# KhutornoyYaroslav/vcm-ts

Measured on AMD Instinct MI355X. Metric: encoded frames/sec at 1920x1080 GOP-32, higher is better.
Workload: dtype f32 (fp16x3 split-MFMA, fp32 accumulate)

## Files before the change

include/dcvc_hip.h:

```cpp
#ifndef DCVC_HIP_H
#define DCVC_HIP_H

#include <stdint.h>

#ifdef __cplusplus
extern "C" {
#endif

#define DCVC_OK 0
#define DCVC_E_ARG (-1)
#define DCVC_E_LAUNCH (-2)
#define DCVC_E_RANGE (-3)

#define DCVC_STATUS_ACT_SATURATED 1

#define DCVC_MAX_SEG 3

#define DCVC_PREC_FP32 0
#define DCVC_PREC_FP16X3 1

typedef struct {
    const float *ptr;
    int32_t C;
    int32_t cs;
} dcvc_seg;

typedef struct {
    dcvc_seg seg[DCVC_MAX_SEG];
    int32_t nseg;
    int32_t N, Hin, Win;
    int32_t in_act;
    float in_slope;
    const float *wpack;
    const float *bpack;
    int32_t ks;
    int32_t stride;
    int32_t Cout;
    int32_t Cout_pad;
    float *out;
    int32_t out_cs;
    int32_t out_act;
    float out_slope;
    int32_t pixel_shuffle;
    const float *res;
    int32_t res_cs;
    const float *res_gate;
    const float *res2;
    int32_t res2_cs;
    int32_t precision;
    int32_t *status;
    float *chan_partial;
    int32_t tile_row0;
    int32_t tile_rows;
    int32_t pair_taps;
} dcvc_conv_args;

int32_t dcvc_conv_tile_rows(int32_t ks, int32_t stride);

int32_t dcvc_conv_chan_partial_parts(int32_t ks, int32_t stride, int32_t Hout, int32_t Wout);
int dcvc_channel_mean_finish(const float *chan_partial, int32_t parts, int32_t row_stride, float *mean, int32_t N,
                             int32_t C, int32_t HW, void *stream);

int64_t dcvc_conv_pack_size(int32_t Cout, int32_t ks, int32_t nseg, const int32_t *seg_C, int32_t *cout_pad);

int dcvc_conv_pack_weights(const float *w, const float *b, int32_t Cout, int32_t ks, int32_t nseg,
                           const int32_t *seg_C, int32_t pixel_shuffle, int32_t precision, float *wpack,
                           float *bpack);

int64_t dcvc_conv_pack_size_paired(int32_t Cout, int32_t Cin, int32_t *cout_pad);
int dcvc_conv_pack_weights_paired(const float *w, const float *b, int32_t Cout, int32_t Cin, float *wpack, float *bpack);

int dcvc_conv2d(const dcvc_conv_args *a, void *stream);
int dcvc_conv_set_lookahead(int32_t mode);

int64_t dcvc_conv_small_pack_bytes(int32_t Cout, int32_t ks, int32_t nseg, const int32_t *seg_C);
int dcvc_conv_small_pack_weights(const float *w, const float *b, int32_t Cout, int32_t ks, int32_t nseg,
                                 const int32_t *seg_C, void *wpack, float *bpack);
int dcvc_conv2d_small(const dcvc_conv_args *a, void *stream);

int64_t dcvc_conv_k32_pack_bytes(int32_t Cout, int32_t ks, int32_t nseg, const int32_t *seg_C, int32_t *cout_pad);
int dcvc_conv_k32_pack_weights(const float *w, const float *b, int32_t Cout, int32_t ks, int32_t nseg,
                               const int32_t *seg_C, int32_t pixel_shuffle, void *wpack, float *bpack);
int dcvc_conv2d_k32(const dcvc_conv_args *a, void *stream);
int dcvc_conv_k32_set_waves(int32_t waves);

int dcvc_warp(const float *src, int32_t src_cs, const float *flow, int32_t flow_cs, float *out, int32_t out_cs,
              int32_t N, int32_t H, int32_t W, int32_t C, void *stream);
int dcvc_up2(const float *src, int32_t src_cs, float *out, int32_t out_cs, float *out2, int32_t out2_cs,
             int32_t N, int32_t H, int32_t W, int32_t C, float scale, void *stream);
int dcvc_down2(const float *src, int32_t src_cs, float *out, int32_t out_cs, int32_t N, int32_t H, int32_t W,
               int32_t C, float scale, int32_t avgpool_order, void *stream);
int dcvc_maxpool2(const float *src, int32_t src_cs, float *out, int32_t out_cs, int32_t N, int32_t H, int32_t W,
                  int32_t C, void *stream);
int dcvc_copy_channels(const float *src, int32_t src_cs, float *out, int32_t out_cs, int64_t npix, int32_t C,
                       void *stream);
int dcvc_nchw_to_nhwc(const float *src, float *out, int32_t out_cs, int32_t N, int32_t C, int32_t H, int32_t W,
                      void *stream);
int dcvc_nhwc_to_nchw(const float *src, int32_t src_cs, float *out, int32_t N, int32_t C, int32_t H, int32_t W,
                      int32_t clamp01, void *stream);

int dcvc_channel_mean(const float *src, int32_t src_cs, float *mean, float *scratch, int32_t N, int32_t HW,
                      int32_t C, void *stream);
int dcvc_se_gate(const float *mean, const float *w1, const float *w2, float *gate, int32_t N, int32_t C,
                 int32_t Cr, void *stream);

int dcvc_scale_channels(const float *src, int32_t src_cs, float *out, int32_t out_cs, const float *q_basic,
                        const float *q_scale, int32_t mode, int32_t N, int32_t HW, int32_t C, void *stream);
int dcvc_scale_channels_map(const float *src, int32_t src_cs, float *out, int32_t out_cs, const float *q_basic,
                            const float *q_scale, int32_t mode, int32_t N, int32_t HW, int32_t C, const float *q_map,
                            int32_t H, int32_t W, void *stream);
int dcvc_round_symbols(const float *z, int32_t z_cs, float *z_hat, int32_t zh_cs, int32_t *sym, int32_t N,
                       int32_t H, int32_t W, int32_t C, void *stream);
int dcvc_symbols_to_nhwc(const int32_t *sym, float *out, int32_t out_cs, int32_t N, int32_t H, int32_t W,
                         int32_t C, void *stream);

typedef struct {
    const float *y;
    int32_t y_cs;
    const float *fusion;
    int32_t fusion_cs;
    const float *spatial;
    int32_t spatial_cs;
    float *params;
    int32_t params_cs;
    float *y_hat;
    float *y_q;
    float *y_res;
    float *scales_hat;
    int32_t *sym;
    int32_t *idx;
    float *out;
    int32_t out_cs;
    const float *q_basic;
    const float *q_scale;
    int32_t N, H, W, C;
    int32_t step;
    const float *idx_edges;
    const float *forced_q;
    const float *q_map;
} dcvc_dual_prior_args;

int dcvc_scale_indexes(const float *scales, int32_t *idx, int64_t n, const float *idx_edges, void *stream);

int dcvc_dual_prior_enc(const dcvc_dual_prior_args *a, void *stream);
int dcvc_dual_prior_dec_index(const dcvc_dual_prior_args *a, void *stream);
int dcvc_dual_prior_dec_apply(const dcvc_dual_prior_args *a, void *stream);

int dcvc_scale_bits(const float *y_q, const float *scales_hat, float *out, float *scratch, int32_t kind, int32_t N,
                    int64_t per_sample, void *stream);
int dcvc_factorized_bits(const float *z_hat, int32_t z_cs, const float *params, float *out, float *scratch, int32_t N,
                         int32_t HW, int32_t C, void *stream);
int dcvc_sq_err(const float *a, int32_t a_cs, const float *b, int32_t b_cs, float *out, float *scratch, int32_t N,
                int32_t HW, int32_t C, void *stream);

int32_t dcvc_cdf_table_cols(void);
int dcvc_build_scale_cdfs(const float *scales, int32_t n_scales, int32_t kind, int32_t *cdf, int32_t *sizes,
                          int32_t *offsets, void *stream);
int dcvc_build_factorized_cdfs(const float *params, int32_t C, int32_t *cdf, int32_t *sizes, int32_t *offsets, void *stream);

const char *dcvc_hip_version(void);

#ifdef __cplusplus
}
#endif
#endif
```

vcm_ts_amd/csrc/conv_k32.hip:

```cpp
#include <hip/hip_runtime.h>
#include <math.h>
#include <stdint.h>
#include <stdlib.h>
#include <string.h>

#include "dcvc_hip.h"
#include "kernel_common.h"


namespace {

constexpr int KC = 32;
constexpr int REC = 40;

struct K32 {
    const float *seg_ptr[DCVC_MAX_SEG];
    int seg_C[DCVC_MAX_SEG];
    int seg_cs[DCVC_MAX_SEG];
    int nseg;
    int H, W;
    int in_act;
    float in_slope;
    const float *wpack;
    const float *bpack;
    int Cout, Cout_pad;
    float *out;
    int out_cs;
    int out_act;
    float out_slope;
    int ps;
    const float *res;
    int res_cs;
    const float *res_gate;
    const float *res2;
    int res2_cs;
    int *status;
    float *chan_partial;
    int ntx;
    int ty0, nty, band_rows;
};

template <int KS, int NTW, int NWAVE>
__global__ __launch_bounds__(64 * NWAVE, NWAVE / 2) void conv_k32(const K32 a) {
    constexpr int NTH = 64 * NWAVE, RW = 8 / NWAVE, MT = 2 * RW;

    constexpr int BH = 8, BW = 32, BN = 16 * NTW;
    constexpr int PH = BH + KS - 1, PW = BW + KS - 1, PAD = KS / 2;
    constexpr int T = KS * KS, TPS = KS, NST = KS;
    constexpr int LDS_MAIN = PH * PW * REC + TPS * 8 * BN * 4;
    static_assert(LDS_MAIN >= 8 * BN, "the SE reduction reuses the front of the buffer");
    __shared__ __attribute__((aligned(16))) float lds[LDS_MAIN];
    float *patch = lds;
    float *wl = lds + PH * PW * REC;

    const int tid = threadIdx.x, lane = tid & 63, wave = tid >> 6;
    const int nbn = a.Cout_pad / BN;
    const int nb = blockIdx.x % nbn, tx = blockIdx.x / nbn;
    const int ty = blockIdx.y + a.ty0;
    const int x0 = tx * BW, y0 = ty * BH, n0 = nb * BN, img = blockIdx.z;

    f32x4 acc[MT][NTW];
#pragma unroll
    for (int m = 0; m < MT; ++m)
#pragma unroll
        for (int n = 0; n < NTW; ++n) acc[m][n] = (f32x4){0.f, 0.f, 0.f, 0.f};

    const int a_base = ((wave * RW) * PW + (lane & 15)) * REC + (lane >> 4) * 4;
    const int b_base = ((lane >> 4) * BN + (lane & 15)) * 4;

    constexpr int NP = (PH * PW * 8 + NTH - 1) / NTH, NW = (TPS * 8 * BN + NTH - 1) / NTH;
    f32x4 rp[NP], rw[NW];
    struct Cursor {
        int s, c0, cg, st;
    };
    auto advance = [&](Cursor &k) {
        if (++k.st == NST) {
            k.st = 0;
            ++k.cg;
            k.c0 += KC;
            if (k.c0 >= a.seg_C[k.s]) {
                ++k.s;
                k.c0 = 0;
            }
        }
    };
    static_assert((PH * PW * 241 < (1 << 23) && PW == 34) || KS != 3, "the multiply-shift below divides by PW = 34");
    auto ld16 = [](const void *base, unsigned byte_off) __attribute__((always_inline)) {
        return *(const f32x4 *)((const char *)base + byte_off);
    };
    static_assert((PH * PW) % 4 == 0, "slot_pixel permutes inside groups of four pixels");
    auto slot_pixel = [](int q) __attribute__((always_inline)) { return (q & ~3) | ((q & 1) << 1) | ((q >> 1) & 1); };
    auto load_patch = [&](const Cursor &k) {
        const unsigned cs4 = (unsigned)a.seg_cs[k.s] * 4u;
        const char *sp = (const char *)(a.seg_ptr[k.s] + (size_t)img * a.H * a.W * a.seg_cs[k.s] + k.c0);
        int t = tid;
        asm volatile("" : "+v"(t));
        const unsigned lane_off = (t & 7) * 16u;
        const unsigned img_bytes = (unsigned)(a.H * a.W) * cs4;
        const __amdgpu_buffer_rsrc_t rs = __builtin_amdgcn_make_buffer_rsrc((void *)sp, 0, (int)img_bytes, 0x00020000);
#pragma unroll
        for (int u = 0; u < NP; ++u) {
            const int i = t + u * NTH;
            const int p = slot_pixel(i >> 3);
            const int py = PW == 34 ? (p * 241) >> 13 : p / PW, px = p - py * PW;
            const int gy = y0 - PAD + py, gx = x0 - PAD + px;
            const unsigned ok = (unsigned)(tid + u * NTH < PH * PW * 8) & (unsigned)((unsigned)gy < (unsigned)a.H) &
                                (unsigned)((unsigned)gx < (unsigned)a.W);
            const unsigned off = ok ? __umul24((unsigned)(gy * a.W + gx), cs4) + lane_off : img_bytes;
            rp[u] = __builtin_bit_cast(f32x4, __builtin_amdgcn_raw_buffer_load_b128(rs, (int)off, 0, 0));
        }
    };
    auto store_patch = [&]() {
#pragma unroll
        for (int u = 0; u < NP; ++u) {
            const int i = tid + u * NTH;
            if (i < PH * PW * 8) {
                f32x4 sv = rp[u] * ACT_SCALE;
                if (a.in_act) {
#pragma unroll
                    for (int e = 0; e < 4; ++e) {
                        const float t = sv[e] * a.in_slope;
                        float r;
                        asm("v_max_f32 %0, %1, %2" : "=v"(r) : "v"(sv[e]), "v"(t));
                        sv[e] = r;
                    }
                }
#pragma unroll
                for (int e = 0; e < 4; ++e) sv[e] = __builtin_amdgcn_fmed3f(sv[e], -F16_MAX, F16_MAX);
                const f16x4 hi = __builtin_convertvector(sv, f16x4);
                const f16x4 lo = __builtin_convertvector(sv - __builtin_convertvector(hi, f32x4), f16x4);
                _Float16 *rec = (_Float16 *)&patch[slot_pixel(i >> 3) * REC];
                *(f16x4 *)&rec[(i & 7) * 4] = hi;
                *(f16x4 *)&rec[32 + (i & 7) * 4] = lo;
            }
        }
    };
    auto load_w = [&](const Cursor &k) {
        const char *wsrc = (const char *)(a.wpack + ((size_t)(k.cg * T + k.st * TPS) * 8) * a.Cout_pad * 4 + (size_t)n0 * 4);
        int t = tid;
        asm volatile("" : "+v"(t));
#pragma unroll
        for (int u = 0; u < NW; ++u) {
            const int i = t + u * NTH;
            if (u + 1 < NW || tid + u * NTH < TPS * 8 * BN) rw[u] = ld16(wsrc, (unsigned)((i / BN) * a.Cout_pad + (i % BN)) * 16u);
        }
    };
    auto store_w = [&]() {
#pragma unroll
        for (int u = 0; u < NW; ++u) {
            const int i = tid + u * NTH;
            if (i < TPS * 8 * BN) *(f32x4 *)&wl[i * 4] = rw[u];
        }
    };

    auto mfma_step = [&](int st) __attribute__((always_inline)) {
        const int a_st = st * PW * REC;
#pragma unroll
        for (int tl = 0; tl < TPS; ++tl) {
            f16x8 ah[MT], al[MT], bh[NTW], bl[NTW];
#pragma unroll
            for (int m = 0; m < MT; ++m) {
                const float *rec = &patch[a_base + a_st + ((m >> 1) * PW + (m & 1) * 16 + tl) * REC];
                ah[m] = *(const f16x8 *)rec;
                al[m] = *(const f16x8 *)(rec + 16);
            }
#pragma unroll
            for (int n = 0; n < NTW; ++n) {
                bh[n] = *(const f16x8 *)&wl[b_base + ((tl * 2 + 0) * 4 * BN + n * 16) * 4];
                bl[n] = *(const f16x8 *)&wl[b_base + ((tl * 2 + 1) * 4 * BN + n * 16) * 4];
            }
#pragma unroll
            for (int m = 0; m < MT; ++m)
#pragma unroll
                for (int n = 0; n < NTW; ++n) {
                    acc[m][n] = __builtin_amdgcn_mfma_f32_16x16x32_f16(bh[n], ah[m], acc[m][n], 0, 0, 0);
                    acc[m][n] = __builtin_amdgcn_mfma_f32_16x16x32_f16(bl[n], ah[m], acc[m][n], 0, 0, 0);
                    acc[m][n] = __builtin_amdgcn_mfma_f32_16x16x32_f16(bh[n], al[m], acc[m][n], 0, 0, 0);
                }
        }
    };

    Cursor cur = {0, 0, 0, 0};
    load_patch(cur);
    load_w(cur);
    while (cur.s < a.nseg) {
        __syncthreads();
        if (cur.st == 0) store_patch();
        store_w();
        __syncthreads();
        Cursor nxt = cur;
        advance(nxt);
        if (cur.st == 0) {
            Cursor nc = cur;
            nc.c0 += KC;
            if (nc.c0 >= a.seg_C[nc.s]) {
                ++nc.s;
                nc.c0 = 0;
            }
            if (nc.s < a.nseg) load_patch(nc);
        }
        if (nxt.s < a.nseg) load_w(nxt);
        mfma_step(cur.st);
        cur = nxt;
    }

    const int Cq = a.Cout >> 2;
    const int Cfin = a.ps ? Cq : a.Cout;
    const int Ho = a.ps ? a.H * 2 : a.H, Wo = a.ps ? a.W * 2 : a.W;
    constexpr float inv_scale = 1.f / (ACT_SCALE * WGT_SCALE);
    int oy[MT], ox[MT];
    unsigned okm = 0;
#pragma unroll
    for (int m = 0; m < MT; ++m) {
        oy[m] = y0 + wave * RW + (m >> 1);
        ox[m] = x0 + (m & 1) * 16 + (lane & 15);
#pragma unroll
        for (int n = 0; n < NTW; ++n)
            if (oy[m] < a.H && ox[m] < a.W && n0 + n * 16 + (lane >> 4) * 4 < a.Cout) okm |= 1u << (m * NTW + n);
    }
    unsigned pixo[MT];
#pragma unroll
    for (int m = 0; m < MT; ++m) pixo[m] = a.ps ? (unsigned)((2 * oy[m]) * Wo + 2 * ox[m]) : (unsigned)(oy[m] * a.W + ox[m]);
    unsigned chq[NTW], pso[NTW];
#pragma unroll
    for (int n = 0; n < NTW; ++n) {
        const int ch = n0 + n * 16 + (lane >> 4) * 4;
        const int sub = a.ps ? ch / Cq : 0;
        chq[n] = (unsigned)(ch - sub * Cq);
        pso[n] = (unsigned)((sub >> 1) * Wo + (sub & 1));
    }
    auto out_off = [&](int m, int n, int cs) __attribute__((always_inline)) -> unsigned {
        return (__umul24(pixo[m] + pso[n], (unsigned)cs) + chq[n]) * 4u;
    };
    const size_t img_pix = (size_t)img * Ho * Wo;
    const char *res_b = a.res ? (const char *)(a.res + img_pix * a.res_cs) : nullptr;
    const char *res2_b = a.res2 ? (const char *)(a.res2 + img_pix * a.res2_cs) : nullptr;
    char *out_b = (char *)(a.out + img_pix * a.out_cs);
    f32x4 rv[MT][NTW];
    const unsigned out_bytes = (unsigned)(Ho * Wo) * (unsigned)a.out_cs * 4u, res_bytes = (unsigned)(Ho * Wo) * (unsigned)a.res_cs * 4u;
    const __amdgpu_buffer_rsrc_t rs_out = __builtin_amdgcn_make_buffer_rsrc((void *)out_b, 0, (int)out_bytes, 0x00020000);
    const __amdgpu_buffer_rsrc_t rs_res = __builtin_amdgcn_make_buffer_rsrc((void *)res_b, 0, a.res ? (int)res_bytes : 0, 0x00020000);
    if (a.res) {
#pragma unroll
        for (int m = 0; m < MT; ++m)
#pragma unroll
            for (int n = 0; n < NTW; ++n) {
                const bool ok = (okm >> (m * NTW + n)) & 1u;
                rv[m][n] = __builtin_bit_cast(f32x4, __builtin_amdgcn_raw_buffer_load_b128(rs_res, (int)(ok ? out_off(m, n, a.res_cs) : res_bytes), 0, 0));
            }
    }
    f32x4 csum[RW][NTW];
    float vmax = 0.f;
#pragma unroll
    for (int n = 0; n < NTW; ++n) {
#pragma unroll
        for (int r = 0; r < RW; ++r) csum[r][n] = (f32x4){0.f, 0.f, 0.f, 0.f};
        const int ch = n0 + n * 16 + (lane >> 4) * 4;
        const f32x4 bias = *(const f32x4 *)&a.bpack[ch];
        f32x4 gate = {1.f, 1.f, 1.f, 1.f};
        if (a.res_gate && ch < a.Cout) gate = *(const f32x4 *)&a.res_gate[(size_t)img * Cfin + (a.ps ? ch % Cq : ch)];
#pragma unroll
        for (int m = 0; m < MT; ++m) {
            f32x4 v = acc[m][n] * inv_scale + bias;
            if (a.out_act == 1) {
                v[0] = act(v[0], a.out_slope);
                v[1] = act(v[1], a.out_slope);
                v[2] = act(v[2], a.out_slope);
                v[3] = act(v[3], a.out_slope);
            } else if (a.out_act == 2) {
#pragma unroll
                for (int e = 0; e < 4; ++e) v[e] = fminf(fmaxf(v[e], 0.f), 1.f);
            }
            if (a.res) {
                if (a.res_gate) {
#pragma unroll
                    for (int e = 0; e < 4; ++e) v[e] = __builtin_fmaf(rv[m][n][e], gate[e], v[e]);
                } else {
                    v = v + rv[m][n];
                }
            }
            const bool ok = (okm >> (m * NTW + n)) & 1u;
            if (!a.res2 && !a.chan_partial) {
                const float m4 = fmaxf(fmaxf(fabsf(v[0]), fabsf(v[1])), fmaxf(fabsf(v[2]), fabsf(v[3])));
                vmax = fmaxf(vmax, ok ? m4 : 0.f);
                __builtin_amdgcn_raw_buffer_store_b128(__builtin_bit_cast(__attribute__((ext_vector_type(4))) int, v), rs_out,
                                                       (int)(ok ? out_off(m, n, a.out_cs) : out_bytes), 0, 0);
            } else if (ok) {
                if (a.res2) v = ld16(res2_b, out_off(m, n, a.res2_cs)) + v;
                if (a.chan_partial) csum[m >> 1][n] += v;
                vmax = fmaxf(vmax, fmaxf(fmaxf(fabsf(v[0]), fabsf(v[1])), fmaxf(fabsf(v[2]), fabsf(v[3]))));
                *(f32x4 *)(out_b + out_off(m, n, a.out_cs)) = v;
            }
        }
    }
    if (a.status && !(vmax <= ACT_LIMIT)) atomicOr(a.status, DCVC_STATUS_ACT_SATURATED);
    if (a.chan_partial) {
#pragma unroll
        for (int r = 0; r < RW; ++r)
#pragma unroll
            for (int n = 0; n < NTW; ++n)
#pragma unroll
                for (int off = 1; off < 16; off <<= 1)
#pragma unroll
                    for (int e = 0; e < 4; ++e) csum[r][n][e] += __shfl_xor(csum[r][n][e], off);
        float *red = lds;
        __syncthreads();
        if ((lane & 15) == 0)
#pragma unroll
            for (int r = 0; r < RW; ++r)
#pragma unroll
                for (int n = 0; n < NTW; ++n) *(f32x4 *)&red[(wave * RW + r) * BN + n * 16 + (lane >> 4) * 4] = csum[r][n];
        __syncthreads();
        if (tid < BN && n0 + tid < a.Cout_pad) {
            float s = red[tid];
#pragma unroll
            for (int w = 1; w < BH; ++w) s += red[w * BN + tid];
            const size_t part = (size_t)img * (a.nty * a.ntx) + (size_t)ty * a.ntx + tx;
            a.chan_partial[part * a.Cout_pad + n0 + tid] = s;
        }
    }
}

template <int KS, int NTW, int NWAVE>
int launch(K32 &k, int N, hipStream_t st) {
    constexpr int BN = 16 * NTW;
    k.ntx = (k.W + 31) / 32;
    k.nty = (k.H + 7) / 8;
    if (k.ty0 < 0 || k.ty0 >= k.nty) return DCVC_E_ARG;
    const int rows = k.band_rows > 0 ? (k.band_rows < k.nty - k.ty0 ? k.band_rows : k.nty - k.ty0) : k.nty;
    dim3 grid((unsigned)(k.ntx * (k.Cout_pad / BN)), (unsigned)rows, (unsigned)N);
    hipLaunchKernelGGL((conv_k32<KS, NTW, NWAVE>), grid, dim3(64 * NWAVE), 0, st, k);
    RET_LAUNCH();
}

int g_k32_waves = 8;

}

extern "C" int64_t dcvc_conv_k32_pack_bytes(int32_t Cout, int32_t ks, int32_t nseg, const int32_t *seg_C, int32_t *cout_pad) {
    if (Cout <= 0 || nseg <= 0 || nseg > DCVC_MAX_SEG || (ks != 1 && ks != 3)) return DCVC_E_ARG;
    int chunks = 0;
    for (int s = 0; s < nseg; ++s) {
        if (seg_C[s] <= 0 || seg_C[s] % KC) return DCVC_E_ARG;
        chunks += seg_C[s] / KC;
    }
    const int cp = round_up(Cout, 32);
    if (cout_pad) *cout_pad = cp;
    return (int64_t)chunks * ks * ks * 8 * cp * 16;
}

extern "C" int dcvc_conv_k32_pack_weights(const float *w, const float *b, int32_t Cout, int32_t ks, int32_t nseg,
                                          const int32_t *seg_C, int32_t pixel_shuffle, void *wpack, float *bpack) {
    int32_t cp = 0;
    const int64_t total = dcvc_conv_k32_pack_bytes(Cout, ks, nseg, seg_C, &cp);
    if (total < 0 || (pixel_shuffle && (Cout & 3))) return DCVC_E_ARG;
    const int T = ks * ks;
    int Cin = 0;
    for (int s = 0; s < nseg; ++s) Cin += seg_C[s];
    memset(wpack, 0, (size_t)total);
    memset(bpack, 0, (size_t)cp * sizeof(float));
    _Float16 *base = (_Float16 *)wpack;
    const int Cq = Cout / 4;
    bool clamped = false;
    for (int c = 0; c < Cin; ++c) {
        const int cg = c / KC, kq = (c % KC) >> 3, j = c & 7;
        for (int t = 0; t < T; ++t)
            for (int n = 0; n < Cout; ++n) {
                const int np = pixel_shuffle ? ps_packed_channel(n, Cq) : n;
                float sv = w[((size_t)n * Cin + c) * T + t] * WGT_SCALE;
                if (!(fabsf(sv) <= F16_MAX)) { clamped = true; sv = sv > 0.f ? F16_MAX : -F16_MAX; }
                const SplitF16 p = split_f16(sv);
                base[(((((size_t)cg * T + t) * 2 + 0) * 4 + kq) * cp + np) * 8 + j] = p.hi;
                base[(((((size_t)cg * T + t) * 2 + 1) * 4 + kq) * cp + np) * 8 + j] = p.lo;
            }
    }
    for (int n = 0; n < Cout; ++n) bpack[pixel_shuffle ? ps_packed_channel(n, Cq) : n] = b ? b[n] : 0.f;
    return clamped ? DCVC_E_RANGE : DCVC_OK;
}

extern "C" int dcvc_conv_k32_set_waves(int32_t waves) {
    if (waves != 4 && waves != 8) return DCVC_E_ARG;
    g_k32_waves = waves;
    return DCVC_OK;
}

extern "C" int dcvc_conv2d_k32(const dcvc_conv_args *a, void *stream) {
    if (!conv_args_ok(a)) return DCVC_E_ARG;
    if (a->stride != 1 || (a->ks != 1 && a->ks != 3) || a->precision != DCVC_PREC_FP16X3) return DCVC_E_ARG;
    if (a->Cout_pad % 32 || a->Cout > a->Cout_pad || (a->pixel_shuffle && (a->Cout & 3))) return DCVC_E_ARG;
    if (a->out_act < 0 || a->out_act > 2) return DCVC_E_ARG;
    for (int s = 0; s < a->nseg; ++s)
        if (a->seg[s].C <= 0 || a->seg[s].C % KC) return DCVC_E_ARG;
    {
        const unsigned long long opix = (unsigned long long)a->Hin * a->Win * (a->pixel_shuffle ? 4 : 1);
        if (opix >= (1ull << 24) || (unsigned long long)a->out_cs * 4ull >= (1ull << 24) ||
            (a->res && (unsigned long long)a->res_cs * 4ull >= (1ull << 24)) ||
            (a->res2 && (unsigned long long)a->res2_cs * 4ull >= (1ull << 24)))
            return DCVC_E_ARG;
        for (int s = 0; s < a->nseg; ++s)
            if ((unsigned long long)a->seg[s].cs * 4ull >= (1ull << 24)) return DCVC_E_ARG;
        if (opix * a->out_cs * 4ull > 0xfffffff0ull || (a->res && opix * a->res_cs * 4ull > 0xfffffff0ull) ||
            (a->res2 && opix * a->res2_cs * 4ull > 0xfffffff0ull))
            return DCVC_E_ARG;
    }
    if (a->in_act && !(a->in_slope >= 0.f && a->in_slope <= 1.f)) return DCVC_E_ARG;
    for (int s = 0; s < a->nseg; ++s)
        if ((unsigned long long)a->Hin * a->Win * a->seg[s].cs * 4ull > 0xfffffff0ull) return DCVC_E_ARG;
    if (!vec_epilogue_ok(a)) return DCVC_E_ARG;
    if (a->chan_partial && a->pixel_shuffle) return DCVC_E_ARG;
    K32 k;
    memset(&k, 0, sizeof(k));
    copy_conv_args_full(k, a);
    k.H = a->Hin;
    k.W = a->Win;
    hipStream_t st = (hipStream_t)stream;
    const bool wide = (a->Cout_pad % 64) == 0;
    const bool w8 = g_k32_waves != 4;
    if (a->ks == 3) return wide ? (w8 ? launch<3, 4, 8>(k, a->N, st) : launch<3, 4, 4>(k, a->N, st)) : launch<3, 2, 4>(k, a->N, st);
    return wide ? launch<1, 4, 4>(k, a->N, st) : launch<1, 2, 4>(k, a->N, st);
}
```

vcm_ts_amd/lib.py:

```python
from __future__ import annotations

import ctypes as C
import functools
import os

HERE = os.path.dirname(os.path.abspath(__file__))
CSRC = os.path.join(HERE, "csrc")


class LibraryMissing(RuntimeError):
    pass


class KernelError(RuntimeError):
    pass


def _load(name):
    path = os.environ.get("DCVC_HIP_LIB") if name == "libdcvc_hip.so" and os.environ.get("DCVC_HIP_LIB") else \
        os.path.join(CSRC, name)
    if not os.path.exists(path):
        raise LibraryMissing(f"{path} not built; run `make -C {CSRC}` (no CPU fallback exists)")
    return C.CDLL(path)


@functools.lru_cache(maxsize=None)
def rans():
    L = _load("libdcvc_rans.so")
    L.dcvc_rans_encoder_create.restype = C.c_void_p
    L.dcvc_rans_encoder_destroy.argtypes = [C.c_void_p]
    L.dcvc_rans_encoder_reset.argtypes = [C.c_void_p]
    L.dcvc_rans_encoder_encode_with_indexes.argtypes = [C.c_void_p, C.c_void_p, C.c_void_p, C.c_int64, C.c_void_p,
                                                        C.c_int32, C.c_int32, C.c_void_p, C.c_void_p]
    L.dcvc_rans_encoder_flush_bound.argtypes = [C.c_void_p]
    L.dcvc_rans_encoder_flush_bound.restype = C.c_int64
    L.dcvc_rans_encoder_flush.argtypes = [C.c_void_p, C.c_void_p, C.c_int64]
    L.dcvc_rans_encoder_flush.restype = C.c_int64
    L.dcvc_rans_decoder_create.restype = C.c_void_p
    L.dcvc_rans_decoder_destroy.argtypes = [C.c_void_p]
    L.dcvc_rans_decoder_set_stream.argtypes = [C.c_void_p, C.c_char_p, C.c_int64]
    L.dcvc_rans_decoder_decode_stream.argtypes = [C.c_void_p, C.c_void_p, C.c_int64, C.c_void_p, C.c_int32,
                                                  C.c_int32, C.c_void_p, C.c_void_p, C.c_void_p]
    L.dcvc_pmf_to_quantized_cdf.argtypes = [C.c_void_p, C.c_int32, C.c_int32, C.c_void_p]
    return L


class Seg(C.Structure):
    _fields_ = [("ptr", C.c_void_p), ("C", C.c_int32), ("cs", C.c_int32)]


class ConvArgs(C.Structure):
    _fields_ = [
        ("seg", Seg * 3), ("nseg", C.c_int32), ("N", C.c_int32), ("Hin", C.c_int32), ("Win", C.c_int32),
        ("in_act", C.c_int32), ("in_slope", C.c_float), ("wpack", C.c_void_p), ("bpack", C.c_void_p),
        ("ks", C.c_int32), ("stride", C.c_int32), ("Cout", C.c_int32), ("Cout_pad", C.c_int32),
        ("out", C.c_void_p), ("out_cs", C.c_int32), ("out_act", C.c_int32), ("out_slope", C.c_float),
        ("pixel_shuffle", C.c_int32), ("res", C.c_void_p), ("res_cs", C.c_int32), ("res_gate", C.c_void_p),
        ("res2", C.c_void_p), ("res2_cs", C.c_int32), ("precision", C.c_int32), ("status", C.c_void_p),
        ("chan_partial", C.c_void_p), ("tile_row0", C.c_int32), ("tile_rows", C.c_int32), ("pair_taps", C.c_int32),
    ]


class DualPriorArgs(C.Structure):
    _fields_ = [
        ("y", C.c_void_p), ("y_cs", C.c_int32), ("fusion", C.c_void_p), ("fusion_cs", C.c_int32),
        ("spatial", C.c_void_p), ("spatial_cs", C.c_int32), ("params", C.c_void_p), ("params_cs", C.c_int32),
        ("y_hat", C.c_void_p), ("y_q", C.c_void_p), ("y_res", C.c_void_p), ("scales_hat", C.c_void_p),
        ("sym", C.c_void_p), ("idx", C.c_void_p), ("out", C.c_void_p), ("out_cs", C.c_int32),
        ("q_basic", C.c_void_p), ("q_scale", C.c_void_p), ("N", C.c_int32), ("H", C.c_int32), ("W", C.c_int32),
        ("C", C.c_int32), ("step", C.c_int32), ("idx_edges", C.c_void_p), ("forced_q", C.c_void_p),
        ("q_map", C.c_void_p),
    ]


class ConvBwdArgs(C.Structure):
    _fields_ = [
        ("dout", C.c_void_p), ("dout_cs", C.c_int32), ("out", C.c_void_p), ("out_cs", C.c_int32),
        ("res", C.c_void_p), ("res_cs", C.c_int32), ("gate", C.c_void_p), ("res2", C.c_void_p), ("res2_cs", C.c_int32),
        ("dres", C.c_void_p), ("dres_cs", C.c_int32), ("dres2", C.c_void_p), ("dres2_cs", C.c_int32),
        ("dpre", C.c_void_p), ("dpre_cs", C.c_int32), ("zs", C.c_int32), ("Hd", C.c_int32), ("Wd", C.c_int32),
        ("N", C.c_int32), ("Ho", C.c_int32), ("Wo", C.c_int32), ("Cout", C.c_int32), ("pixel_shuffle", C.c_int32),
        ("act", C.c_int32), ("slope", C.c_float),
    ]


class WgradArgs(C.Structure):
    _fields_ = [
        ("x", C.c_void_p), ("x_cs", C.c_int32), ("C", C.c_int32), ("in_act", C.c_int32), ("in_slope", C.c_float),
        ("dpre", C.c_void_p), ("dpre_cs", C.c_int32), ("zs", C.c_int32), ("Hd", C.c_int32), ("Wd", C.c_int32),
        ("N", C.c_int32), ("Hin", C.c_int32), ("Win", C.c_int32), ("Ho", C.c_int32), ("Wo", C.c_int32),
        ("Cout", C.c_int32), ("ks", C.c_int32), ("stride", C.c_int32), ("dw", C.c_void_p), ("Cin_total", C.c_int32),
        ("cin_offset", C.c_int32), ("scratch", C.c_void_p), ("scratch_floats", C.c_int64), ("overwrite", C.c_int32),
        ("db", C.c_void_p), ("precision", C.c_int32),
    ]


class PackJob(C.Structure):
    _fields_ = [
        ("w", C.c_void_p), ("b", C.c_void_p), ("Cout", C.c_int32), ("Cin_total", C.c_int32), ("ks", C.c_int32),
        ("nseg", C.c_int32), ("seg_C", C.c_int32 * 3), ("cin_offset", C.c_int32), ("pixel_shuffle", C.c_int32),
        ("precision", C.c_int32), ("transposed", C.c_int32), ("wpack", C.c_void_p), ("bpack", C.c_void_p),
    ]


class DualPriorBwdArgs(C.Structure):
    _fields_ = [
        ("y", C.c_void_p), ("y_cs", C.c_int32), ("fusion", C.c_void_p), ("fusion_cs", C.c_int32),
        ("y_hat", C.c_void_p), ("dout", C.c_void_p), ("dout_cs", C.c_int32), ("dy_res", C.c_void_p),
        ("dscales_hat", C.c_void_p), ("dparams", C.c_void_p), ("dparams_cs", C.c_int32),
        ("dspatial", C.c_void_p), ("dspatial_cs", C.c_int32), ("dy", C.c_void_p), ("dy_cs", C.c_int32),
        ("dfusion", C.c_void_p), ("dfusion_cs", C.c_int32), ("dq_plane", C.c_void_p),
        ("q_basic", C.c_void_p), ("q_scale", C.c_void_p), ("N", C.c_int32), ("H", C.c_int32), ("W", C.c_int32),
        ("C", C.c_int32), ("step", C.c_int32),
    ]


class ColorCoeffs(C.Structure):
    _fields_ = [(n, C.c_float) for n in ("y_off", "c_off", "y_scale", "c_scale", "crr", "cgb", "cgr", "cbb", "kr", "kg", "kb",
                                         "icb", "icr", "y_range", "c_range")] + \
               [(n, C.c_int32) for n in ("max_code", "bit_depth", "siting", "matrix", "range")]


class RoiBox(C.Structure):
    _fields_ = [(n, C.c_int32) for n in ("x1", "y1", "x2", "y2", "cls")]


class RoiClassRec(C.Structure):
    _fields_ = [("border", C.c_int32), ("shrink", C.c_int32), ("feather", C.c_float * 64)]


PRECISIONS = {"fp32": 0, "fp16x3": 1}

i32, i64, f32, vp = C.c_int32, C.c_int64, C.c_float, C.c_void_p

HEADERS = {
    "dcvc_hip.h": {
        "dcvc_conv_tile_rows": (i32, i32, i32),
        "dcvc_conv_chan_partial_parts": (i32, i32, i32, i32, i32),
        "dcvc_channel_mean_finish": [vp, i32, i32, vp, i32, i32, i32, vp],
        "dcvc_conv_pack_size": (i64, i32, i32, i32, vp, C.POINTER(i32)),
        "dcvc_conv_pack_weights": [vp, vp, i32, i32, i32, vp, i32, i32, vp, vp],
        "dcvc_conv_pack_size_paired": (i64, i32, i32, C.POINTER(i32)),
        "dcvc_conv_pack_weights_paired": [vp, vp, i32, i32, vp, vp],
        "dcvc_conv2d": [C.POINTER(ConvArgs), vp],
        "dcvc_conv_set_lookahead": [i32],
        "dcvc_conv_small_pack_bytes": (i64, i32, i32, i32, vp),
        "dcvc_conv_small_pack_weights": [vp, vp, i32, i32, i32, vp, vp, vp],
        "dcvc_conv2d_small": [C.POINTER(ConvArgs), vp],
        "dcvc_conv_k32_pack_bytes": (i64, i32, i32, i32, vp, C.POINTER(i32)),
        "dcvc_conv_k32_pack_weights": [vp, vp, i32, i32, i32, vp, i32, vp, vp],
        "dcvc_conv2d_k32": [C.POINTER(ConvArgs), vp],
        "dcvc_conv_k32_set_waves": [i32],
        "dcvc_warp": [vp, i32, vp, i32, vp, i32, i32, i32, i32, i32, vp],
        "dcvc_up2": [vp, i32, vp, i32, vp, i32, i32, i32, i32, i32, f32, vp],
        "dcvc_down2": [vp, i32, vp, i32, i32, i32, i32, i32, f32, i32, vp],
        "dcvc_maxpool2": [vp, i32, vp, i32, i32, i32, i32, i32, vp],
        "dcvc_copy_channels": [vp, i32, vp, i32, i64, i32, vp],
        "dcvc_nchw_to_nhwc": [vp, vp, i32, i32, i32, i32, i32, vp],
        "dcvc_nhwc_to_nchw": [vp, i32, vp, i32, i32, i32, i32, i32, vp],
        "dcvc_channel_mean": [vp, i32, vp, vp, i32, i32, i32, vp],
        "dcvc_se_gate": [vp, vp, vp, vp, i32, i32, i32, vp],
        "dcvc_scale_channels": [vp, i32, vp, i32, vp, vp, i32, i32, i32, i32, vp],
        "dcvc_scale_channels_map": [vp, i32, vp, i32, vp, vp, i32, i32, i32, i32, vp, i32, i32, vp],
        "dcvc_round_symbols": [vp, i32, vp, i32, vp, i32, i32, i32, i32, vp],
        "dcvc_symbols_to_nhwc": [vp, vp, i32, i32, i32, i32, i32, vp],
        "dcvc_scale_indexes": [vp, vp, i64, vp, vp],
        "dcvc_dual_prior_enc": [C.POINTER(DualPriorArgs), vp],
        "dcvc_dual_prior_dec_index": [C.POINTER(DualPriorArgs), vp],
        "dcvc_dual_prior_dec_apply": [C.POINTER(DualPriorArgs), vp],
        "dcvc_scale_bits": [vp, vp, vp, vp, i32, i32, i64, vp],
        "dcvc_factorized_bits": [vp, i32, vp, vp, vp, i32, i32, i32, vp],
        "dcvc_sq_err": [vp, i32, vp, i32, vp, vp, i32, i32, i32, vp],
        "dcvc_cdf_table_cols": (i32,),
        "dcvc_build_scale_cdfs": [vp, i32, i32, vp, vp, vp, vp],
        "dcvc_build_factorized_cdfs": [vp, i32, vp, vp, vp, vp],
        "dcvc_hip_version": (C.c_char_p,),
    },
    "dcvc_hip_grad.h": {
        "dcvc_conv_pack_weights_dev": [vp, vp, i32, i32, i32, i32, vp, i32, i32, i32, i32, vp, vp, vp],
        "dcvc_pack_plan_create": [C.POINTER(PackJob), i32, C.POINTER(C.c_void_p)],
        "dcvc_pack_plan_run": [vp, vp],
        "dcvc_pack_plan_destroy": (None, vp),
        "dcvc_conv_bwd_prologue": [C.POINTER(ConvBwdArgs), vp],
        "dcvc_conv_wgrad_scratch_min": (i64, i32, i32, i32),
        "dcvc_conv_wgrad": [C.POINTER(WgradArgs), vp],
        "dcvc_channel_dot": [vp, i32, vp, i32, vp, vp, i32, i32, i32, i32, i32, vp],
        "dcvc_mask_accumulate": [vp, i32, vp, i32, f32, vp, i32, i64, i32, vp],
        "dcvc_add_planes": [vp, i32, vp, i32, vp, i32, i64, i32, vp],
        "dcvc_warp_bwd": [vp, i32, vp, i32, vp, i32, vp, i32, vp, i32, i32, i32, i32, i32, vp, vp],
        "dcvc_up2_bwd": [vp, i32, vp, i32, i32, i32, i32, i32, f32, vp],
        "dcvc_down2_bwd": [vp, i32, vp, i32, i32, i32, i32, i32, f32, vp],
        "dcvc_maxpool2_bwd": [vp, i32, vp, i32, vp, i32, i32, i32, i32, i32, vp],
        "dcvc_se_bwd": [vp, vp, vp, vp, vp, vp, vp, vp, i32, i32, i32, vp],
        "dcvc_add_channel_vec": [vp, i32, vp, f32, i32, i32, i32, vp],
        "dcvc_scale_channels_bwd": [vp, i32, vp, i32, vp, vp, i32, i32, i32, i32, vp],
        "dcvc_q_finish": [vp, vp, vp, vp, vp, vp, i32, i32, vp],
        "dcvc_dual_prior_bwd": [C.POINTER(DualPriorBwdArgs), vp],
        "dcvc_scale_bits_bwd": [vp, vp, vp, vp, vp, i32, i32, i64, vp],
        "dcvc_factorized_bits_bwd": [vp, i32, vp, vp, vp, i32, vp, i32, i32, i32, vp],
        "dcvc_sq_err_bwd": [vp, i32, vp, i32, vp, vp, i32, i32, i32, i32, vp],
    },
    "dcvc_hip_rans.h": {
        "dcvc_drans_default_lanes": (i32, i64),
        "dcvc_drans_scratch_words": (i64, i64, i32),
        "dcvc_drans_build_lut": [vp, i32, i32, vp, vp],
        "dcvc_drans_encode": [vp, vp, i32, i32, i64, vp, i32, i32, vp, vp, i32, vp, i64, vp, i64, vp, vp, vp, vp],
        "dcvc_drans_decode": [vp, i64, vp, vp, vp, i32, i32, i64, vp, i32, i32, vp, vp, vp, i32, vp, vp, vp],
    },
    "dcvc_hip_metrics.h": {
        "dcvc_ms_ssim": [vp, vp, i32, i32, i32, i32, i32, i64, i32, i64, f32, i32, vp, vp, vp, vp, vp],
        "dcvc_ms_ssim_grad": [vp, vp, i32, i32, i32, i32, i32, i64, i32, i64, f32, i32, vp, vp, vp, vp],
        "dcvc_ms_ssim_workspace_bytes": (i64, i32, i32, i32, i32, i32),
    },
    "dcvc_hip_color.h": {
        "dcvc_color_coeffs": [i32, i32, i32, i32, vp],
        "dcvc_yuv420_to_rgb": [vp, vp, vp, i32, i32, i32, i32, vp, vp, i32, i32, i32, i64, i32, vp],
        "dcvc_rgb_to_yuv420": [vp, i32, i32, i32, i64, vp, vp, vp, vp, i32, i32, vp, vp, vp, i32, i32, vp, vp],
    },
    "dcvc_hip_roi.h": {
        "dcvc_roi_residual": [vp, i32, i64, vp, i32, i64, i32, i32, vp, vp, i32, vp, i64, i64, i32, i32, i32, i32, vp],
        "dcvc_roi_fuse": [vp, i32, i64, vp, i64, i64, i32, i32, i32, i32, i32, i32, vp, vp, i32, vp, i32, vp, i32, i64, vp],
        "dcvc_roi_sse": [vp, i32, i64, vp, i32, i64, i32, i32, vp, vp, i32, vp, i32, vp, vp],
        "dcvc_roi_qmap": [i32, i32, vp, vp, i32, i32, vp, i32, vp, vp],
    },
    "dcvc_hip_roil.h": {
        "dcvc_roil_cells": [i32, i32, vp, i32, vp, vp, i32],
        "dcvc_roil_check": [vp, i64, vp, i32],
        "dcvc_roil_encode": [vp, i32, i64, vp, i32, i64, i32, i32, vp, vp, i32, i32, vp, i32, vp, vp, i64, vp, vp],
        "dcvc_roil_decode": [vp, vp, i64, i32, i32, vp, vp, i32, vp, vp, i64, i64, i32, i32, i32, i32, vp, vp],
    },
    "dcvc_hip_scene.h": {"dcvc_scene_hist": [vp, i32, i64, i32, i32, vp, vp]},
    "dcvc_hip_bits.h": {
        "dcvc_bits_map_scale": [vp, vp, vp, vp, vp, i32, i32, vp, vp, vp, i32, i32, i32, i32, vp, vp],
        "dcvc_bits_map_factorized": [vp, vp, i32, i32, vp, vp, vp, i32, i32, i32, i32, vp, vp],
        "dcvc_bits_regions": [vp, vp, i32, vp, i32, i32, i32, vp, vp],
        "dcvc_bits_sweep_scale": [vp, vp, vp, vp, i32, vp, i32, i32, vp, vp, vp, i32, i32, i32, i32, vp, vp],
    },
    "dcvc_hip_hash.h": {
        "dcvc_hash_pixels": [vp, i32, i64, i32, i32, vp, vp, vp],
        "dcvc_hash_f32": [vp, i32, i64, i32, i32, i32, vp, vp, vp],
    },
    "dcvc_hip_scale.h": {"dcvc_scale_planes": [vp, i32, i64, vp, i32, i64, i32, i32, i32, i32, i32, vp, vp, vp, vp, i32, vp, vp, vp, vp, i32, vp]},
    "dcvc_hip_aq.h": {
        "dcvc_aq_activity": [vp, i32, i64, i32, i32, vp, vp, vp],
        "dcvc_aq_map": [vp, vp, i32, i32, vp, vp, vp, vp, vp],
    },
    "dcvc_hip_motion.h": {"dcvc_motion_step": [vp, i32, i64, i32, i32, vp, i32, i32, i32, i32, vp, vp]},
    "dcvc_hip_tnr.h": {"dcvc_tnr_step": [vp, i32, i64, vp, i32, i64, vp, i32, i64, i32, i32, vp, i32, vp, vp, vp]},
    "dcvc_hip_redact.h": {"dcvc_redact": [vp, i32, i64, vp, i32, i64, i32, i32, vp, vp, i32, i32, i32, i32, i32, vp, vp]},
    "dcvc_hip_me.h": {
        "dcvc_me_search": [vp, i32, i64, vp, i32, i64, i32, i32, i32, i32, vp, vp, vp, vp],
        "dcvc_me_compensate": [vp, i32, i64, vp, i32, i64, i32, i32, vp, vp],
    },
    "dcvc_hip_png.h": {
        "dcvc_png_bound": (i64, i32, i32, i32),
        "dcvc_png_tables_check": [vp, i32],
        "dcvc_png_encode": [vp, i32, i64, i32, i32, i32, vp, vp, i32, vp, vp, i64, vp, vp],
    },
    "dcvc_hip_grain.h": {
        "dcvc_grain_measure": [vp, i32, i64, vp, i32, i64, i32, i32, vp, vp, vp],
        "dcvc_grain_apply": [vp, i32, i64, vp, i32, i64, i32, i32, i32, i32, i32, vp, vp],
    },
    "dcvc_hip_tnr_fuse.h": {
        "dcvc_tnr_fuse": [vp, i32, i64, vp, vp, vp, vp, i32, i64, i32, vp, i32, i64, i32, i32, vp, vp, i32, vp, vp, vp],
    },
    "dcvc_hip_mesub.h": {
        "dcvc_me_refine": [vp, i32, i64, vp, i32, i64, i32, i32, i32, vp, vp, vp, vp],
        "dcvc_me_compensate_sub": [vp, i32, i64, vp, i32, i64, i32, i32, vp, vp],
    },
    "dcvc_hip_mesplit.h": {
        "dcvc_me_split": [vp, i32, i64, vp, i32, i64, i32, i32, i32, i32, vp, vp, vp, vp],
        "dcvc_me_compensate_split": [vp, i32, i64, vp, i32, i64, i32, i32, vp, vp],
    },
    "dcvc_hip_mepyr.h": {
        "dcvc_me_pyramid": [vp, i32, i64, i32, i32, i32, vp, i32, vp, i32, vp, i32, vp],
        "dcvc_me_coarse": [vp, i32, vp, i32, i32, i32, i32, i32, i32, vp, vp],
        "dcvc_me_descend": [vp, i32, vp, i32, i32, i32, i32, i32, i32, i32, vp, vp, vp, vp, vp],
    },
    "dcvc_hip_deint.h": {
        "dcvc_deinterlace420": [vp, vp, vp, i32, i32, vp, vp, vp, i32, i32, vp, vp, vp, i32, i32, i32, i32, i32, i32, i32, vp, vp, vp, i32, i32,
                                vp, i32, vp],
    },
    "dcvc_hip_noise.h": {
        "dcvc_noise_cells": [vp, i32, i64, i32, i32, vp, vp, i32, vp, vp],
        "dcvc_noise_hist": [vp, i64, vp, vp],
    },
}


def _signature(entry):
    return (entry[0], list(entry[1:])) if isinstance(entry, tuple) else (C.c_int, entry)


ALL_HIP_SYMBOLS = [name for funcs in HEADERS.values() for name in funcs]
_SIGS = {name: _signature(e)[1] for funcs in HEADERS.values() for name, e in funcs.items() if isinstance(e, list) or e[0] is None}
_CORE = ("dcvc_hip.h", "dcvc_hip_grad.h", "dcvc_hip_rans.h")
HIP_SYMBOLS = sorted(name for h in _CORE for name in HEADERS[h])
(METRICS_SYMBOLS, COLOR_SYMBOLS, ROI_SYMBOLS, ROIL_SYMBOLS, SCENE_SYMBOLS, BITS_SYMBOLS, HASH_SYMBOLS, SCALE_SYMBOLS, AQ_SYMBOLS,
 MOTION_SYMBOLS, TNR_SYMBOLS, REDACT_SYMBOLS, ME_SYMBOLS, PNG_SYMBOLS, GRAIN_SYMBOLS, TNR_FUSE_SYMBOLS, MESUB_SYMBOLS, MESPLIT_SYMBOLS,
 MEPYR_SYMBOLS, DEINT_SYMBOLS, NOISE_SYMBOLS) = (list(funcs) for h, funcs in HEADERS.items() if h not in _CORE)
HASH_CONSTANTS = ["dcvc_hash_chunk_bytes", "dcvc_hash_block_bytes", "dcvc_hash_scratch_bytes"]
RANS_SYMBOLS = [
    "dcvc_rans_encoder_create", "dcvc_rans_encoder_destroy", "dcvc_rans_encoder_reset",
    "dcvc_rans_encoder_encode_with_indexes", "dcvc_rans_encoder_flush_bound", "dcvc_rans_encoder_flush",
    "dcvc_rans_decoder_create", "dcvc_rans_decoder_destroy", "dcvc_rans_decoder_set_stream",
    "dcvc_rans_decoder_decode_stream", "dcvc_pmf_to_quantized_cdf",
]


@functools.lru_cache(maxsize=None)
def hip():
    L = _load("libdcvc_hip.so")
    for funcs in HEADERS.values():
        for name, entry in funcs.items():
            fn = getattr(L, name)
            fn.restype, fn.argtypes = _signature(entry)
    return L


def hash_constant(name):
    return int(i32.in_dll(hip(), name).value)


def check(code, what):
    if code != 0:
        raise KernelError(f"{what} failed with status {code}")
```

Measured before the change: 42.95.

## Unroll 3x3 k32 conv chunk loop with patch prefetch one chunk ahead

```diff
diff --git a/include/dcvc_hip.h b/include/dcvc_hip.h
--- a/include/dcvc_hip.h
+++ b/include/dcvc_hip.h
@@ -83,6 +83,7 @@
                                const int32_t *seg_C, int32_t pixel_shuffle, void *wpack, float *bpack);
 int dcvc_conv2d_k32(const dcvc_conv_args *a, void *stream);
 int dcvc_conv_k32_set_waves(int32_t waves);
+int dcvc_conv_k32_set_lookahead(int32_t mode);
 
 int dcvc_warp(const float *src, int32_t src_cs, const float *flow, int32_t flow_cs, float *out, int32_t out_cs,
               int32_t N, int32_t H, int32_t W, int32_t C, void *stream);
diff --git a/vcm_ts_amd/csrc/conv_k32.hip b/vcm_ts_amd/csrc/conv_k32.hip
--- a/vcm_ts_amd/csrc/conv_k32.hip
+++ b/vcm_ts_amd/csrc/conv_k32.hip
@@ -3,6 +3,7 @@
 #include <stdint.h>
 #include <stdlib.h>
 #include <string.h>
+#include <type_traits>
 
 #include "dcvc_hip.h"
 #include "kernel_common.h"
@@ -40,8 +41,8 @@
     int ty0, nty, band_rows;
 };
 
-template <int KS, int NTW, int NWAVE>
-__global__ __launch_bounds__(64 * NWAVE, NWAVE / 2) void conv_k32(const K32 a) {
+template <int KS, int NTW, int NWAVE, bool AHEAD>
+__device__ __forceinline__ void conv_k32_tile(const K32 &a) {
     constexpr int NTH = 64 * NWAVE, RW = 8 / NWAVE, MT = 2 * RW;
 
     constexpr int BH = 8, BW = 32, BN = 16 * NTW;
@@ -69,6 +70,8 @@
     const int b_base = ((lane >> 4) * BN + (lane & 15)) * 4;
 
     constexpr int NP = (PH * PW * 8 + NTH - 1) / NTH, NW = (TPS * 8 * BN + NTH - 1) / NTH;
+    static_assert(!AHEAD || NST == 3, "AHEAD: the three steps of a 3x3 chunk, written out");
+    static_assert((TPS * 8 * BN) % NTH == 0, "a filter row is a whole number of float4 per thread");
     f32x4 rp[NP], rw[NW];
     struct Cursor {
         int s, c0, cg, st;
@@ -110,29 +113,37 @@
             rp[u] = __builtin_bit_cast(f32x4, __builtin_amdgcn_raw_buffer_load_b128(rs, (int)off, 0, 0));
         }
     };
+    auto store_slot = [&](const int u, const bool in_act, const int t) __attribute__((always_inline)) {
+        const int i = t + u * NTH;
+        if (tid + u * NTH < PH * PW * 8) {
+            f32x4 sv = rp[u] * ACT_SCALE;
+            if (in_act) {
+#pragma unroll
+                for (int e = 0; e < 4; ++e) {
+                    const float t = sv[e] * a.in_slope;
+                    float r;
+                    asm("v_max_f32 %0, %1, %2" : "=v"(r) : "v"(sv[e]), "v"(t));
+                    sv[e] = r;
+                }
+            }
+#pragma unroll
+            for (int e = 0; e < 4; ++e) sv[e] = __builtin_amdgcn_fmed3f(sv[e], -F16_MAX, F16_MAX);
+            const f16x4 hi = __builtin_convertvector(sv, f16x4);
+            const f16x4 lo = __builtin_convertvector(sv - __builtin_convertvector(hi, f32x4), f16x4);
+            _Float16 *rec = (_Float16 *)&patch[slot_pixel(i >> 3) * REC];
+            *(f16x4 *)&rec[(i & 7) * 4] = hi;
+            *(f16x4 *)&rec[32 + (i & 7) * 4] = lo;
+        }
+    };
     auto store_patch = [&]() {
-#pragma unroll
-        for (int u = 0; u < NP; ++u) {
-            const int i = tid + u * NTH;
-            if (i < PH * PW * 8) {
-                f32x4 sv = rp[u] * ACT_SCALE;
-                if (a.in_act) {
-#pragma unroll
-                    for (int e = 0; e < 4; ++e) {
-                        const float t = sv[e] * a.in_slope;
-                        float r;
-                        asm("v_max_f32 %0, %1, %2" : "=v"(r) : "v"(sv[e]), "v"(t));
-                        sv[e] = r;
-                    }
-                }
-#pragma unroll
-                for (int e = 0; e < 4; ++e) sv[e] = __builtin_amdgcn_fmed3f(sv[e], -F16_MAX, F16_MAX);
-                const f16x4 hi = __builtin_convertvector(sv, f16x4);
-                const f16x4 lo = __builtin_convertvector(sv - __builtin_convertvector(hi, f32x4), f16x4);
-                _Float16 *rec = (_Float16 *)&patch[slot_pixel(i >> 3) * REC];
-                *(f16x4 *)&rec[(i & 7) * 4] = hi;
-                *(f16x4 *)&rec[32 + (i & 7) * 4] = lo;
-            }
+        int t = tid;
+        if (AHEAD) asm volatile("" : "+v"(t));
+        if (AHEAD && a.in_act) {
+#pragma unroll
+            for (int u = 0; u < NP; ++u) store_slot(u, true, t);
+        } else {
+#pragma unroll
+            for (int u = 0; u < NP; ++u) store_slot(u, !AHEAD && a.in_act, t);
         }
     };
     auto load_w = [&](const Cursor &k) {
@@ -142,14 +153,14 @@
 #pragma unroll
         for (int u = 0; u < NW; ++u) {
             const int i = t + u * NTH;
-            if (u + 1 < NW || tid + u * NTH < TPS * 8 * BN) rw[u] = ld16(wsrc, (unsigned)((i / BN) * a.Cout_pad + (i % BN)) * 16u);
+            if (AHEAD || u + 1 < NW || tid + u * NTH < TPS * 8 * BN) rw[u] = ld16(wsrc, (unsigned)((i / BN) * a.Cout_pad + (i % BN)) * 16u);
         }
     };
     auto store_w = [&]() {
 #pragma unroll
         for (int u = 0; u < NW; ++u) {
             const int i = tid + u * NTH;
-            if (i < TPS * 8 * BN) *(f32x4 *)&wl[i * 4] = rw[u];
+            if (AHEAD || i < TPS * 8 * BN) *(f32x4 *)&wl[i * 4] = rw[u];
         }
     };
 
@@ -183,25 +194,62 @@
     Cursor cur = {0, 0, 0, 0};
     load_patch(cur);
     load_w(cur);
-    while (cur.s < a.nseg) {
-        __syncthreads();
-        if (cur.st == 0) store_patch();
-        store_w();
-        __syncthreads();
-        Cursor nxt = cur;
-        advance(nxt);
-        if (cur.st == 0) {
+    if constexpr (AHEAD) {
+        auto chunk = [&](auto more, const Cursor &nc) __attribute__((always_inline)) {
+            constexpr bool MORE = decltype(more)::value;
+            __syncthreads();
+            store_patch();
+            store_w();
+            __syncthreads();
+            advance(cur);
+            load_w(cur);
+            if (MORE) load_patch(nc);
+            __builtin_amdgcn_sched_barrier(0);
+            mfma_step(0);
+            __syncthreads();
+            store_w();
+            __syncthreads();
+            advance(cur);
+            load_w(cur);
+            __builtin_amdgcn_sched_barrier(0);
+            mfma_step(1);
+            __syncthreads();
+            store_w();
+            __syncthreads();
+            if (MORE) load_w(nc);
+            __builtin_amdgcn_sched_barrier(0);
+            mfma_step(2);
+        };
+        for (;;) {
             Cursor nc = cur;
-            nc.c0 += KC;
-            if (nc.c0 >= a.seg_C[nc.s]) {
-                ++nc.s;
-                nc.c0 = 0;
-            }
-            if (nc.s < a.nseg) load_patch(nc);
-        }
-        if (nxt.s < a.nseg) load_w(nxt);
-        mfma_step(cur.st);
-        cur = nxt;
+            nc.st = NST - 1;
+            advance(nc);
+            if (nc.s >= a.nseg) break;
+            chunk(std::true_type{}, nc);
+            cur = nc;
+        }
+        chunk(std::false_type{}, cur);
+    } else {
+        while (cur.s < a.nseg) {
+            __syncthreads();
+            if (cur.st == 0) store_patch();
+            store_w();
+            __syncthreads();
+            Cursor nxt = cur;
+            advance(nxt);
+            if (cur.st == 0) {
+                Cursor nc = cur;
+                nc.c0 += KC;
+                if (nc.c0 >= a.seg_C[nc.s]) {
+                    ++nc.s;
+                    nc.c0 = 0;
+                }
+                if (nc.s < a.nseg) load_patch(nc);
+            }
+            if (nxt.s < a.nseg) load_w(nxt);
+            mfma_step(cur.st);
+            cur = nxt;
+        }
     }
 
     const int Cq = a.Cout >> 2;
@@ -322,6 +370,17 @@
 }
 
 template <int KS, int NTW, int NWAVE>
+__global__ __launch_bounds__(64 * NWAVE, NWAVE / 2) void conv_k32(const K32 a) {
+    conv_k32_tile<KS, NTW, NWAVE, KS == 3>(a);
+}
+template <int KS, int NTW, int NWAVE>
+__global__ __launch_bounds__(64 * NWAVE, NWAVE / 2) void conv_k32_step(const K32 a) {
+    conv_k32_tile<KS, NTW, NWAVE, false>(a);
+}
+
+int g_k32_lookahead = 2;
+
+template <int KS, int NTW, int NWAVE>
 int launch(K32 &k, int N, hipStream_t st) {
     constexpr int BN = 16 * NTW;
     k.ntx = (k.W + 31) / 32;
@@ -329,6 +388,12 @@
     if (k.ty0 < 0 || k.ty0 >= k.nty) return DCVC_E_ARG;
     const int rows = k.band_rows > 0 ? (k.band_rows < k.nty - k.ty0 ? k.band_rows : k.nty - k.ty0) : k.nty;
     dim3 grid((unsigned)(k.ntx * (k.Cout_pad / BN)), (unsigned)rows, (unsigned)N);
+    if constexpr (KS == 3) {
+        if (g_k32_lookahead != 2) {
+            hipLaunchKernelGGL((conv_k32_step<KS, NTW, NWAVE>), grid, dim3(64 * NWAVE), 0, st, k);
+            RET_LAUNCH();
+        }
+    }
     hipLaunchKernelGGL((conv_k32<KS, NTW, NWAVE>), grid, dim3(64 * NWAVE), 0, st, k);
     RET_LAUNCH();
 }
@@ -384,6 +449,12 @@
     return DCVC_OK;
 }
 
+extern "C" int dcvc_conv_k32_set_lookahead(int32_t mode) {
+    if (mode != 1 && mode != 2) return DCVC_E_ARG;
+    g_k32_lookahead = mode;
+    return DCVC_OK;
+}
+
 extern "C" int dcvc_conv2d_k32(const dcvc_conv_args *a, void *stream) {
     if (!conv_args_ok(a)) return DCVC_E_ARG;
     if (a->stride != 1 || (a->ks != 1 && a->ks != 3) || a->precision != DCVC_PREC_FP16X3) return DCVC_E_ARG;
diff --git a/vcm_ts_amd/lib.py b/vcm_ts_amd/lib.py
--- a/vcm_ts_amd/lib.py
+++ b/vcm_ts_amd/lib.py
@@ -151,6 +151,7 @@
         "dcvc_conv_k32_pack_weights": [vp, vp, i32, i32, i32, vp, i32, vp, vp],
         "dcvc_conv2d_k32": [C.POINTER(ConvArgs), vp],
         "dcvc_conv_k32_set_waves": [i32],
+        "dcvc_conv_k32_set_lookahead": [i32],
         "dcvc_warp": [vp, i32, vp, i32, vp, i32, i32, i32, i32, i32, vp],
         "dcvc_up2": [vp, i32, vp, i32, vp, i32, i32, i32, i32, i32, f32, vp],
         "dcvc_down2": [vp, i32, vp, i32, i32, i32, i32, i32, f32, i32, vp],
```

Measured after the change: 43.14 (median of 6 runs). Within noise of the previous version (+0.4%).
